# atom501/v-img

Measured on AMD Instinct MI355X. Metric: Mrays/sec (primary+secondary) at 512 spp, higher is better.
Workload: dtype f32; 1 GPU; disney_spheres.json, mis integrator, 512 spp, 1800x800; integrator=mis, spp=512, depth=unbounded, bvh=sweep SAH (host)

## Files before the change

### v-img_amd/csrc/device_scene.h

```cpp
#pragma once
#include <hip/hip_runtime.h>
#include <stdint.h>

#include "../../include/vimg_scene.h"

namespace vimg {

#define VIMG_GLOBAL __attribute__((address_space(1)))
#define VIMG_LDS __attribute__((address_space(3)))
template <typename T>
using gptr = const VIMG_GLOBAL T*;
typedef float v4f __attribute__((ext_vector_type(4)));
typedef uint32_t v2u __attribute__((ext_vector_type(2)));
typedef uint32_t v4u __attribute__((ext_vector_type(4)));

struct __attribute__((aligned(16))) DNode {
  v4f a;
  v4f b;
  v4f c;
  uint32_t left_ref, right_ref, pad0, pad1;
};
static_assert(sizeof(DNode) == 64, "DNode must be one 64-byte line");

struct __attribute__((aligned(16))) DLeafPrim {
  v4f a, b;
  float c0;
  uint32_t prim;
// ... 18 lines not shown

struct DScene {
  float cam_to_world[16];
  float p_size0, p_size1;
  float cone_spread;
  float aperture_radius, focal_dist;
  int32_t res_x, res_y;

  float root_min[3], root_max[3];
  uint32_t num_nodes, max_depth;
  uint32_t root_ref;
  gptr<DNode> nodes;
  gptr<DLeafPrim> leaf_prims;

  gptr<VimgPrim> prims;
  gptr<DTriShade> tri_shade;
  gptr<float> tri_area_pdf;
  gptr<VimgMesh> meshes;
  gptr<float> normals;
  gptr<float> uvs;
  gptr<VimgSphere> spheres;
  gptr<VimgMaterial> materials;
  gptr<uint32_t> material_flags;
  gptr<VimgTexture> textures;
  gptr<float> texels;
  gptr<VimgTextureRG> rg_textures;
  gptr<float> rg_texels;
  gptr<VimgLight> lights;
  gptr<DLight> dlights;
  uint32_t num_lights;
  gptr<float> cdf_pool;
  VimgBackground background;
  uint32_t background_emissive;
};

enum : uint32_t {
  MATF_NEEDS_UV = 1u,
  MATF_NEEDS_FRAME = 2u,
};

struct RenderArgs {
  uint32_t integrator, samples, depth;
  uint32_t tile_rank, tile_world;
  uint32_t tiles_x, tiles_y;
  uint32_t num_local_tiles;
  uint32_t full_stats;
// ... 49 lines not shown
```

### v-img_amd/csrc/hip_internal.h

```cpp
#pragma once
#include <hip/hip_runtime.h>

#include <algorithm>
#include <string>
#include <utility>
#include <vector>

#include "../../include/vimg_hip.h"
#include "device_mem.h"
#include "device_scene.h"
#include "kernel_tus.h"

#pragma GCC visibility push(hidden)
struct VimgDeviceScene {
  vimg::DScene d{};
  vimg::DevBuf nodes, leaf_prims;
  vimg::DevBuf chain_leaf;
  std::vector<vimg::DevBuf> tables;
  size_t total_bytes = 0;
  bool textured = false;
  VimgHipOptions opt{};
  int waves_per_simd = 2;
  bool too_wide = false;
  bool force_general = false;
  uint32_t num_cus = 0;
  uint32_t num_leaf_prims = 0;
  vimg::DevBuf stats;
  vimg::DevBuf counter;
  vimg::DevBuf root_box;
  vimg::DevBuf frame;
  vimg::DevBuf pool_cold;
  vimg::DevBuf stack_ovf;
  vimg::DevBuf pool_state;
  uint32_t pool_epoch = 0;
  uint64_t generation = 0;
  uint32_t num_vertices = 0, num_tris = 0, num_spheres = 0;
  std::vector<std::pair<uint32_t, uint32_t>> normal_rows;
  uint32_t n_internal = 0;
  uint32_t n_chain = 0;
  std::vector<uint32_t> level_begin;
  std::vector<VimgMaterial> materials;
  std::vector<VimgTexture> textures;
  std::vector<VimgLight> lights;
  uint32_t num_rg_textures = 0;
  uint64_t num_texels = 0, num_cdf = 0;
  size_t lights_table = 0, dlights_table = 0;
  int query_launch = -1;
  bool query_ready = false;
  vimg::RenderArgs query_args{};
  uint32_t query_lds = 0;
  uint32_t query_per_cu[3] = {0, 0, 0};
};

struct VimgProgressive {
  VimgDeviceScene* scene = nullptr;
  VimgRenderParams params{};
  uint64_t items = 0;
  vimg::DevBuf rec[2];
  int cur = 0;
  uint32_t samples = 0;
  vimg::DevBuf scratch;
  uint64_t generation = 0;
  bool uniform = true;
  uint64_t valid_items = 0;
  uint64_t launches = 0;
  vimg::DevBuf item_list;
  vimg::DevBuf block_counts;
  vimg::DevBuf ctl;
};
// ... 17 lines not shown
  bool deep;
  int cu_waves;
  bool feature;
  size_t cold_bytes;
  size_t ovf_bytes;
};

struct DeviceTree {
  DevBuf nodes, bb, obj_indices;
  uint32_t num_nodes = 0, max_depth = 0;
  std::vector<uint32_t> level_internal;
};
int build_tree_device(uint32_t builder , uint32_t n, const float* d_bounds6, DeviceTree* out);

int validate_materials(const VimgMaterial* materials, uint32_t num_materials, const VimgTexture* textures, uint32_t num_textures,
                       uint32_t num_rg_textures);
int validate_lights(const VimgLight* lights, uint32_t num_lights, uint32_t num_prims);
bool tables_textured(const VimgMaterial* materials, uint32_t num_materials, const VimgTexture* textures, const VimgBackground& bg);
bool background_is_emissive(const VimgBackground& bg);

struct RelightPlan {
  bool any = false;
  DevBuf new_lights, new_dlights;
  DevBuf sin_elev, lum, row_int, row_tot;
  std::vector<float> sin_table;
};
int check_relight(const VimgDeviceScene* s, const VimgGeometryUpdate* u);
int prepare_relight(const VimgDeviceScene* s, const VimgGeometryUpdate* u, RelightPlan* plan);
int enqueue_relight(VimgDeviceScene* s, const VimgGeometryUpdate* u, RelightPlan* plan, hipStream_t st);
void commit_relight(VimgDeviceScene* s, const VimgGeometryUpdate* u, RelightPlan* plan);

struct EnvCdfScratch {
  float* sin_elev;
  float* lum;
  float* row_int;
  float* row_tot;
};
void enqueue_mip_levels(float* texels, const uint64_t* level_offset, uint32_t levels, uint32_t w, uint32_t h, uint32_t wrap_u,
                        uint32_t wrap_v, hipStream_t st);
std::vector<float> env_sin_table(uint32_t h);
void enqueue_env_cdfs(const float* img, uint32_t w, uint32_t h, const EnvCdfScratch& t, float* row_cdf, float* col_cdfs, hipStream_t st);

struct ProgLaunch {
  uint32_t base;
  const void* in;
  void* out;
  const uint32_t* item_list = nullptr;
  uint32_t item_count = 0;
  bool keep_stats = false;
};
int check_params(const VimgDeviceScene* s, const VimgRenderParams* p);
int check_render(const VimgDeviceScene* s, const VimgRenderParams* p, const void* d_out);
struct RenderLaunch {
// ... 25 lines not shown
```

### v-img_amd/csrc/render_kernels.h

```cpp
#pragma once
#include "device_math.h"
#include "device_scene.h"

namespace vimg {


struct Rng {
  uint64_t s;
};
VD uint32_t pcg_next(Rng& r) {
  uint64_t old = r.s;
  r.s = old * 6364136223846793005ULL + 1ULL;
  uint32_t xorshifted = static_cast<uint32_t>(((old >> 18u) ^ old) >> 27u);
  uint32_t rot = static_cast<uint32_t>(old >> 59u);
  return (xorshifted >> rot) | (xorshifted << ((0u - rot) & 31u));
}
VD void pcg_seed(Rng& r, uint64_t initstate) {
  r.s = 0;
  pcg_next(r);
  r.s += initstate;
  pcg_next(r);
}
constexpr uint64_t kPcgA = 6364136223846793005ULL;
constexpr uint64_t pcg_a_pow(int n) { uint64_t r = 1; for (int i = 0; i < n; ++i) r *= kPcgA; return r; }
constexpr uint64_t pcg_c_sum(int n) { uint64_t r = 0; for (int i = 0; i < n; ++i) r += pcg_a_pow(i); return r; }
// ... 736 lines not shown
}

enum : uint32_t {
  LOBE_NONE = 0,
  LOBE_COSINE = 1,
  LOBE_CLEARCOAT = 2,
  LOBE_METAL = 3,
  LOBE_GLASS = 4,
  LOBE_DIELECTRIC = 5
};

VD float fresnel_dielectric(float n_dot_i, float eta) {
  float n_dot_t_sq = 1.f - (1.f - n_dot_i * n_dot_i) / (eta * eta);
  if (n_dot_t_sq < 0) return 1;
  float n_dot_t = sqrt_f(n_dot_t_sq);
  n_dot_i = absf(n_dot_i);
  float rs = (n_dot_i - eta * n_dot_t) / (n_dot_i + eta * n_dot_t);
  float rp = (eta * n_dot_i - n_dot_t) / (eta * n_dot_i + n_dot_t);
  return (rs * rs + rp * rp) / 2;
}
VD float fd_term(f3 n, f3 w, float fd90) {
  return 1.f + (fd90 - 1.f) * pow5(1.f - sel_max(dot(n, w), 0.f));
}
VD void regularize_alpha(float& ax, float& ay) {
  ax = ax < 0.1f ? clampf(2.f * ax, 0.03f, 0.1f) : ax;
  ay = ay < 0.1f ? clampf(2.f * ay, 0.03f, 0.1f) : ay;
}

struct PrincipledCommon {
  f3 dir_in;
  Onb frame;
  float metallic, roughness;
};
template <bool TEX>
VD PrincipledCommon principled_prologue(const DScene& g, gptr<VimgMaterial> m, f3 wi, const Hit& hit) {
  PrincipledCommon p;
  p.dir_in = -wi;
  p.frame = Onb{hit.tu, hit.tv, hit.ns};
  if ((dot(hit.ns, p.dir_in) * dot(hit.ng, p.dir_in)) < 0) {
    p.frame.u = -p.frame.u;
    p.frame.v = -p.frame.v;
    p.frame.w = -p.frame.w;
  }
  f2 m_r{1.f, 1.f};
  if constexpr (TEX) {
    if (m->mr_tex >= 0) m_r = rg_get_at_uv(g, m->mr_tex, hit.mr_uv);
  }
  m_r = m_r * f2{m->metallic_factor, m->roughness_factor};
  p.metallic = m_r.x;
  p.roughness = m_r.y;
  return p;
}

template <bool TEX>
VD void principled_eval_pdf(const DScene& g, gptr<VimgMaterial> m, f3 wi,
                                                 f3 wo, const Hit& hit, RayCone cone,
                                                 bool regularize, f3& f_out, float& pdf_out) {
  const PrincipledCommon pc = principled_prologue<TEX>(g, m, wi, hit);
  const f3 dir_in = pc.dir_in;
  const Onb& frame = pc.frame;
  const float metallic = pc.metallic, roughness = pc.roughness;
  const f3 base_color = col_at_ray_hit<TEX>(g, m->tex, wi, cone, hit);
  const f3 half_vector = normalize(dir_in + wo);
  constexpr float alpha_min = 0.0001;
  const float aspect = sqrt_f(1.f - 0.9f * m->anisotropic);
  const float roughness_clamp = clampf(roughness, 0.01f, 1.f);
  const float roughness_square = roughness_clamp * roughness_clamp;
  float alphax = sel_max(alpha_min, roughness_square / aspect);
  float alphay = sel_max(alpha_min, roughness_square * aspect);
  if (regularize) regularize_alpha(alphax, alphay);
  const float g_in = g_w(dir_in, alphax, alphay, frame);
  const float G = g_in * g_w(wo, alphax, alphay, frame);
  const float ng_in = dot(hit.ng, dir_in);
  const float ng_out = dot(hit.ng, wo);

  f3 eval_glass;
  float pdf_glass;
  {
    const float mat_eta = m->eta;
    float in_geo_dot = dot(dir_in, hit.ng);
    bool reflect = (in_geo_dot * dot(hit.ng, wo)) >= 0;
    float eta = in_geo_dot >= 0 ? mat_eta : 1.f / mat_eta;
    f3 hv = half_vector;
    if (!reflect) hv = normalize(dir_in + wo * eta);
    float h_dot_in = dot(hv, dir_in);
    float F = fresnel_dielectric(h_dot_in, eta);
    const f3 lh = project_onto_onb(frame, hv);
    float had = (lh.x * lh.x) / (alphax * alphax) + (lh.y * lh.y) / (alphay * alphay)
                + (lh.z * lh.z);
    float D = 1. / (kPi * alphax * alphay * (had * had));
    float normal_in_dot = dot(frame.w, dir_in);
    if (reflect) {
      eval_glass = base_color * (F * D * G) / (4.f * absf(normal_in_dot));
      pdf_glass = (F * D * g_in) / (4.f * absf(normal_in_dot));
    } else {
      float eta_factor = 1.f / (eta * eta);
      float h_dot_out = dot(hv, wo);
      float sqrt_denom = h_dot_in + eta * h_dot_out;
      eval_glass = f3{sqrt_f(base_color.x), sqrt_f(base_color.y), sqrt_f(base_color.z)}
                   * (eta_factor * (1 - F) * D * G * eta * eta * absf(h_dot_out * h_dot_in))
                   / (absf(normal_in_dot) * sqrt_denom * sqrt_denom);
      float dh_dout = eta * eta * h_dot_out / (sqrt_denom * sqrt_denom);
      pdf_glass = (1.f - F) * D * g_in * absf(dh_dout * h_dot_in / normal_in_dot);
    }
  }
  const float st = m->specular_transmission;
  if (ng_in < 0) {
    f_out = (1.f - metallic) * st * eval_glass;
    pdf_out = pdf_glass;
    return;
  }
  const bool below = (ng_in < 0 || ng_out < 0);

  f3 eval_sheen{0.f, 0.f, 0.f};
  f3 eval_diff{0.f, 0.f, 0.f};
  float pdf_diff = 0.f;
  f3 eval_clearcoat{0.f, 0.f, 0.f};
  float pdf_clearcoat = 0.f;
  f3 eval_metal{0.f, 0.f, 0.f};
  float pdf_metal = 0.f;

  float alpha_g = (1.f - m->clearcoat_gloss) * 0.1f + m->clearcoat_gloss * 0.001f;
  alpha_g = regularize && (alpha_g < 0.1f) ? clampf(2.f * alpha_g, 0.03f, 0.1f) : alpha_g;

  if (!below) {
    const float base_lum = luminance(base_color);
    const f3 c_tint = base_lum > 0 ? base_color / base_lum : splat3(1.f);
    {
      const float sheen_tint = m->sheen_tint;
      f3 c_sheen = (splat3(1.f) - splat3(sheen_tint)) + sheen_tint * c_tint;
      eval_sheen = c_sheen * pow5(1.f - sel_max(dot(half_vector, wo), 0.f))
                   * sel_max(dot(frame.w, wo), 0.f);
    }
    {
      const float subsurface = m->subsurface;
      float normal_dirout_dot = dot(frame.w, wo);
      const float cos_theta_out = sel_max(normal_dirout_dot, 0.f);
      const float cos_theta_in = sel_max(dot(frame.w, dir_in), 0.f);
      const float dot_h_out = sel_max(dot(half_vector, wo), 0.f);
      const float fd90 = 0.5 + 2.0 * roughness * dot_h_out * dot_h_out;
      const f3 base_diffuse = base_color * kInvPiF * fd_term(frame.w, dir_in, fd90)
                              * fd_term(frame.w, wo, fd90) * cos_theta_out;
      const float fss90 = roughness * dot_h_out * dot_h_out;
      f3 ss_diffuse = base_color * 1.25f * kInvPiF
                      * (fd_term(frame.w, dir_in, fss90) * fd_term(frame.w, wo, fss90)
                             * ((1.f / (cos_theta_out + cos_theta_in)) - 0.5f)
                         + 0.5f)
                      * cos_theta_out;
      eval_diff = (1.f - subsurface) * base_diffuse + subsurface * ss_diffuse;
      pdf_diff = sel_max(normal_dirout_dot, 0.f) * kInvPiF;
    }
    {
      constexpr float R0 = ((1.5f - 1.f) * (1.5f - 1.f)) / ((1.5f + 1.f) * (1.5f + 1.f));
      float h_dirout_dot = absf(dot(half_vector, wo));
      float fresnel = R0 + (1. - R0) * pow5(1.f - h_dirout_dot);
      float Gc = g_w(dir_in, 0.25, 0.25, frame) * g_w(wo, 0.25, 0.25, frame);
      const float ag2 = alpha_g * alpha_g;
      const f3 lh = project_onto_onb(frame, half_vector);
      float D = (ag2 - 1.f) / (kPi * F_log(ag2) * (1. + (ag2 - 1.) * lh.z * lh.z));
      float clearcoat_eval = (fresnel * D * Gc) / (4.f * absf(dot(frame.w, dir_in)));
      pdf_clearcoat = (D * absf(dot(frame.w, half_vector))) / (4.f * h_dirout_dot);
      eval_clearcoat = splat3(clearcoat_eval);
    }
    {
      const float spec_tint = m->specular_tint, specular = m->specular, eta = m->eta;
      f3 k_s = (splat3(1.f) - splat3(spec_tint)) + spec_tint * c_tint;
      float R0 = ((eta - 1.f) * (eta - 1.f)) / ((eta + 1.f) * (eta + 1.f));
      f3 c_0 = (specular * R0 * (1.f - metallic)) * k_s + metallic * base_color;
      f3 fresnel = c_0 + (splat3(1.f) - c_0) * pow5(1.f - dot(half_vector, wo));
      const f3 lh = project_onto_onb(frame, half_vector);
      float had = (lh.x * lh.x) / (alphax * alphax) + (lh.y * lh.y) / (alphay * alphay)
                  + (lh.z * lh.z);
      float D = 1. / (kPi * alphax * alphay * (had * had));
      float d_mul_denominator = D / (4.f * absf(dot(frame.w, dir_in)));
      eval_metal = fresnel * G * d_mul_denominator;
      pdf_metal = g_in * d_mul_denominator;
    }
  }
  const float clearcoat = m->clearcoat, sheen = m->sheen;
  f3 eval_principled = ((1.f - st) * (1.f - metallic) * eval_diff)
                       + ((1.f - metallic) * sheen * eval_sheen)
                       + (0.25f * clearcoat * eval_clearcoat)
                       + ((1.f - st * (1.f - metallic)) * eval_metal)
                       + ((1.f - metallic) * st * eval_glass);
  float diffuse_weight = (1.f - metallic) * (1.f - st);
  float clearcoat_weight = 0.25f * clearcoat;
  float metal_weight = (1.f - st * (1.f - metallic));
  float glass_weight = (1.f - metallic) * st;
  float total_w = diffuse_weight + clearcoat_weight + metal_weight + glass_weight;
  float choose_diff = diffuse_weight / total_w;
  float choose_clearcoat = clearcoat_weight / total_w;
  float choose_metal = metal_weight / total_w;
  float choose_glass = glass_weight / total_w;
  pdf_out = choose_diff * pdf_diff + choose_clearcoat * pdf_clearcoat + choose_metal * pdf_metal
            + choose_glass * pdf_glass;
  f_out = eval_principled;
}

template <bool TEX, int MT = -1>
VD Scatter sample_mat(const DScene& g, const Hit& hit, f3 wi, Rng& rng, bool regularize) {
  gptr<VimgMaterial> m = g.materials + hit.mat;
  const uint32_t type = MT >= 0 ? uint32_t(MT) : m->type;
  const f3 dir_in = -wi;
  uint32_t lobe = LOBE_NONE;
  Onb frame{f3{1.f, 0.f, 0.f}, f3{0.f, 1.f, 0.f}, f3{0.f, 0.f, 1.f}};
  float alphax = 0.f, alphay = 0.f, eta = 0.f, alpha_g = 0.f;
  bool lambert_front = true;

  if (type == VIMG_MAT_LAMBERTIAN) {
    lobe = LOBE_COSINE;
    lambert_front = dot(wi, hit.ns) < 0;
    frame = init_onb(lambert_front ? hit.ns : -hit.ns);
  } else if (type == VIMG_MAT_DIELECTRIC) {
    lobe = LOBE_DIELECTRIC;
  } else if (type == VIMG_MAT_PRINCIPLED) {
    const PrincipledCommon pc = principled_prologue<TEX>(g, m, wi, hit);
    frame = pc.frame;
    const float metallic = pc.metallic;
    float roughness = pc.roughness;
    const float ng_in = dot(hit.ng, dir_in);
    if (ng_in < 0) {
      lobe = LOBE_GLASS;
    } else {
      const float st = m->specular_transmission;
      float diffuse_weight = (1.f - metallic) * (1.f - st);
      float clearcoat_weight = 0.25f * m->clearcoat;
      float metal_weight = (1.f - st * (1.f - metallic));
      float glass_weight = (1.f - metallic) * st;
      float total_w = diffuse_weight + clearcoat_weight + metal_weight + glass_weight;
      float choose_diff = diffuse_weight / total_w;
      float choose_clearcoat = clearcoat_weight / total_w;
      float choose_metal = metal_weight / total_w;
      float choose_glass = glass_weight / total_w;
      float rnd = rand_float(rng);
      if (rnd <= choose_diff) {
        lobe = LOBE_COSINE;
      } else if (rnd > choose_diff && rnd <= (choose_diff + choose_clearcoat)) {
        lobe = LOBE_CLEARCOAT;
      } else if (rnd > (choose_diff + choose_clearcoat)
                 && rnd <= (choose_diff + choose_clearcoat + choose_metal)) {
        lobe = LOBE_METAL;
      } else if (rnd > (choose_diff + choose_clearcoat + choose_metal)
                 && rnd <= (choose_diff + choose_clearcoat + choose_metal + choose_glass)) {
        lobe = LOBE_GLASS;
      }
    }
    if (lobe == LOBE_CLEARCOAT) {
      const float gloss = m->clearcoat_gloss;
      alpha_g = (1.f - gloss) * 0.1f + gloss * 0.001f;
      if (regularize && alpha_g < 0.1f) alpha_g = clampf(2.f * alpha_g, 0.03f, 0.1f);
    } else if (lobe == LOBE_METAL || lobe == LOBE_GLASS) {
      constexpr float alpha_min = 0.0001;
      float aspect = sqrt_f(1.f - 0.9f * m->anisotropic);
      if (lobe == LOBE_GLASS) roughness = clampf(roughness, 0.01f, 1.f);
      float roughness_square = roughness * roughness;
      alphax = sel_max(alpha_min, roughness_square / aspect);
      alphay = sel_max(alpha_min, roughness_square * aspect);
      if (regularize) regularize_alpha(alphax, alphay);
      const float mat_eta = m->eta;
      eta = ng_in >= 0 ? mat_eta : 1.f / mat_eta;
    }
  }
  if (lobe == LOBE_DIELECTRIC) return dielectric_sample(m, hit, wi, rng);
  if (lobe == LOBE_NONE) return no_scatter();

  const float ra = rand_float(rng);
  const float rb = rand_float(rng);
  const float phi = 2 * kPi * ((lobe == LOBE_CLEARCOAT) ? rb : ra);
  double sin_phi, cos_phi;
  sincos_azimuth(phi, sin_phi, cos_phi);

  if (lobe == LOBE_COSINE) {
    float cos_theta = sqrt_f(rb);
    float sin_theta = sqrt_f(1 - cos_theta * cos_theta);
    f3 local{static_cast<float>(cos_phi) * sin_theta, static_cast<float>(sin_phi) * sin_theta,
             cos_theta};
    f3 dir = xform_with_onb(frame, local);
    if (type == VIMG_MAT_LAMBERTIAN) {
      if (lambert_front) return Scatter{dir, 0.f, false, true};
      return no_scatter();
    }
    if (dot(hit.ng, dir) <= 0) return no_scatter();
    return Scatter{dir, 0.f, false, true};
// ... 45 lines not shown
  if (rnd <= F) {
    f3 reflected = normalize(-dir_in + 2 * dot(dir_in, half_vec) * half_vec);
    if (dot(reflected, hit.ng) * dot(dir_in, hit.ng) <= 0) return no_scatter();
    return Scatter{reflected, 0.f, true, true};
  }
  float h_dot_out_sq = 1 - (1 - h_dot_in * h_dot_in) / (eta * eta);
  if (h_dot_out_sq <= 0) return no_scatter();
  if (h_dot_in < 0) half_vec = -half_vec;
  float h_dot_out = static_cast<float>(__builtin_sqrt(static_cast<double>(h_dot_out_sq)));
  f3 refracted = -dir_in / eta + (absf(h_dot_in) / eta - h_dot_out) * half_vec;
  if (dot(refracted, hit.ng) * dot(dir_in, hit.ng) >= 0) return no_scatter();
  f3 generalized_h = normalize(dir_in + refracted * eta);
  float g_h_dot_in = dot(generalized_h, dir_in);
  if ((1 - (1 - g_h_dot_in * g_h_dot_in) / (eta * eta)) <= 0) return no_scatter();
  return Scatter{refracted, eta, true, true};
}
template <bool TEX, int MT = -1>
VD void eval_pdf_pair(const DScene& g, const Hit& hit, f3 wi, f3 wo, RayCone cone, bool regularize,
                      f3& f, float& pdf) {
  gptr<VimgMaterial> m = g.materials + hit.mat;
  const uint32_t type = MT >= 0 ? uint32_t(MT) : m->type;
  if (type == VIMG_MAT_LAMBERTIAN) {
    float dot_product = static_cast<float>(sel_max(0.0f, dot(wo, hit.ns)) / kPi);
    f = col_at_ray_hit<TEX>(g, m->tex, wi, cone, hit) * dot_product;
    pdf = dot_product;
  } else if (type == VIMG_MAT_PRINCIPLED) {
    principled_eval_pdf<TEX>(g, m, wi, wo, hit, cone, regularize, f, pdf);
  } else {
    f = f3{0.f, 0.f, 0.f};
    pdf = 1.0f;
  }
}

VD void tri_light_sample_with(f3 p0, f3 p1, f3 p2, f3 n0, f3 n1, f3 n2, float pdf, f3 look_from, Rng& rng, f3& hit_n,
                              EmitterInfo& info) {
  float rand1 = rand_float(rng);
  float rand2 = rand_float(rng);
  float u, v;
  if (rand1 < rand2) {
    u = rand1 / 2.f;
    v = rand2 - u;
  } else {
    v = rand2 / 2.f;
    u = rand1 - v;
  }
  float w = 1.f - u - v;
  const f3 hit_p = p0 * u + p1 * v + p2 * w;
// ... 630 lines not shown
```

### v-img_amd/csrc/scene_relight.hip

```cpp
#include <hip/hip_runtime.h>

#include <cstring>

#include "device_math.h"
#include "hip_internal.h"
#include "scene_bake.h"

namespace vimg {

namespace {

constexpr uint32_t kBlock = 256;

template <typename T>
VD T* flat(gptr<T> p) {
  return (T*)p;
}

dim3 blocks_for(uint32_t n) { return dim3((n + kBlock - 1) / kBlock); }

}

__global__ void __launch_bounds__(kBlock) scene_relight_flags(const DScene d, uint32_t num_materials) {
  const uint32_t i = blockIdx.x * blockDim.x + threadIdx.x;
  if (i >= num_materials) return;
  flat(d.material_flags)[i] = bake_material_flags(flat(d.materials)[i], flat(d.textures));
}

__global__ void __launch_bounds__(kBlock) scene_relight_cls(const DScene d, uint32_t num_slots) {
  const uint32_t j = blockIdx.x * blockDim.x + threadIdx.x;
  if (j >= num_slots) return;
  DLeafPrim* lp = flat(d.leaf_prims) + j;
  const VimgPrim p = flat(d.prims)[lp->prim];
  lp->cls = bake_material_class(flat(d.materials)[bake_prim_material(p, flat(d.tri_shade), flat(d.meshes), flat(d.spheres))].type);
}

__global__ void __launch_bounds__(kBlock)
scene_relight_lights(const DScene d, const VimgLight* __restrict__ lights, uint32_t num_lights, DLight* __restrict__ out) {
  const uint32_t i = blockIdx.x * blockDim.x + threadIdx.x;
  if (i >= num_lights) return;
  out[i] = bake_light(lights[i], flat(d.prims), flat(d.tri_shade), flat(d.tri_area_pdf), flat(d.meshes), flat(d.spheres), flat(d.materials));
}

namespace {

bool is_env_image(const VimgBackground& bg, uint32_t texture) {
  return bg.type == VIMG_BG_ENVMAP && bg.env_tex >= 0 && static_cast<uint32_t>(bg.env_tex) == texture;
}

bool levels_disjoint(const VimgTexture& t) {
  for (uint32_t a = 0; a < t.num_levels; ++a)
    for (uint32_t b = a + 1; b < t.num_levels; ++b) {
      const uint64_t na = uint64_t(std::max(t.width >> a, 1u)) * std::max(t.height >> a, 1u);
      const uint64_t nb = uint64_t(std::max(t.width >> b, 1u)) * std::max(t.height >> b, 1u);
      if (t.level_offset[a] < t.level_offset[b] + nb && t.level_offset[b] < t.level_offset[a] + na) return false;
    }
  return true;
}

}

int check_relight(const VimgDeviceScene* s, const VimgGeometryUpdate* u) {
  const uint32_t num_textures = static_cast<uint32_t>(s->textures.size());
  if (u->textures)
// ... 22 lines not shown
    if (backgrounds > 1) return fail(VIMG_E_INVALID, "update: more than one background entry in lights");
  }
  if (u->num_images && !u->images) return fail(VIMG_E_INVALID, "update: num_images without images");
  for (uint32_t k = 0; k < u->num_images; ++k) {
    const VimgTextureImage& im = u->images[k];
    if (im.texture >= num_textures || s->textures[im.texture].type != VIMG_TEX_IMAGE)
      return fail(VIMG_E_INVALID, "update: images: texture is not a resident image texture");
    if (!im.level0 || (reinterpret_cast<uintptr_t>(im.level0) & 3u))
      return fail(VIMG_E_INVALID, "update: images: level0 is null or not 4-byte aligned");
    if (!levels_disjoint(s->textures[im.texture]))
      return fail(VIMG_E_UNSUPPORTED, "update: images: the texture's mip levels overlap in the texel pool");
  }
  return VIMG_OK;
}

int prepare_relight(const VimgDeviceScene* s, const VimgGeometryUpdate* u, RelightPlan* plan) {
  plan->any = u->materials || u->textures || u->set_lights || u->background || u->num_images;
  if (!plan->any) return VIMG_OK;
  if (g_device < 0) return fail(VIMG_E_DEVICE, "update: no device");
  if (u->set_lights) {
    if (int rc = plan->new_lights.alloc(std::max<size_t>(u->num_lights, 1) * sizeof(VimgLight))) return rc;
    if (int rc = plan->new_dlights.alloc(std::max<size_t>(u->num_lights, 1) * sizeof(DLight))) return rc;
  }
  for (uint32_t k = 0; k < u->num_images; ++k)
    if (is_env_image(s->d.background, u->images[k].texture) && !plan->lum.p) {
      const VimgTexture& t = s->textures[u->images[k].texture];
      plan->sin_table = env_sin_table(t.height);
      if (int rc = plan->sin_elev.alloc(size_t(t.height) * sizeof(float))) return rc;
      if (int rc = plan->lum.alloc(size_t(t.width) * t.height * sizeof(float))) return rc;
      if (int rc = plan->row_int.alloc(size_t(t.height) * sizeof(float))) return rc;
      if (int rc = plan->row_tot.alloc(sizeof(float))) return rc;
    }
  return VIMG_OK;
}

int enqueue_relight(VimgDeviceScene* s, const VimgGeometryUpdate* u, RelightPlan* plan, hipStream_t st) {
  const DScene& d = s->d;
  float* texels = (float*)d.texels;
  float* cdf_pool = (float*)d.cdf_pool;
  for (uint32_t k = 0; k < u->num_images; ++k) {
    const VimgTextureImage& im = u->images[k];
    const VimgTexture& t = s->textures[im.texture];
    float* level0 = texels + t.level_offset[0] * 3;
    HIP_TRY(hipMemcpyAsync(level0, im.level0, size_t(t.width) * t.height * 3 * sizeof(float), hipMemcpyDeviceToDevice, st));
    enqueue_mip_levels(texels, t.level_offset, t.num_levels, t.width, t.height, t.wrap_u, t.wrap_v, st);
    if (is_env_image(d.background, im.texture)) {
      HIP_TRY(hipMemcpyAsync(plan->sin_elev.p, plan->sin_table.data(), plan->sin_table.size() * sizeof(float), hipMemcpyHostToDevice, st));
      enqueue_env_cdfs(level0, t.width, t.height,
                       EnvCdfScratch{plan->sin_elev.as<float>(), plan->lum.as<float>(), plan->row_int.as<float>(), plan->row_tot.as<float>()},
                       cdf_pool + d.background.row_cdf_offset, cdf_pool + d.background.col_cdf_offset, st);
    }
  }
  if (u->textures && !s->textures.empty())
    HIP_TRY(hipMemcpyAsync((void*)d.textures, u->textures, s->textures.size() * sizeof(VimgTexture), hipMemcpyHostToDevice, st));
  if (u->materials && !s->materials.empty()) {
    const uint32_t n = static_cast<uint32_t>(s->materials.size());
    HIP_TRY(hipMemcpyAsync((void*)d.materials, u->materials, size_t(n) * sizeof(VimgMaterial), hipMemcpyHostToDevice, st));
    hipLaunchKernelGGL(scene_relight_flags, blocks_for(n), dim3(kBlock), 0, st, d, n);
    hipLaunchKernelGGL(scene_relight_cls, blocks_for(s->num_leaf_prims), dim3(kBlock), 0, st, d, s->num_leaf_prims);
  }
  if (u->set_lights) {
    if (u->num_lights) {
      HIP_TRY(hipMemcpyAsync(plan->new_lights.p, u->lights, size_t(u->num_lights) * sizeof(VimgLight), hipMemcpyHostToDevice, st));
      hipLaunchKernelGGL(scene_relight_lights, blocks_for(u->num_lights), dim3(kBlock), 0, st, d, plan->new_lights.as<const VimgLight>(),
                         u->num_lights, plan->new_dlights.as<DLight>());
    }
  } else if (u->materials && d.num_lights) {
    hipLaunchKernelGGL(scene_relight_lights, blocks_for(d.num_lights), dim3(kBlock), 0, st, d, (const VimgLight*)d.lights, d.num_lights,
                       (DLight*)d.dlights);
  }
  HIP_TRY(hipGetLastError());
  return VIMG_OK;
}

void commit_relight(VimgDeviceScene* s, const VimgGeometryUpdate* u, RelightPlan* plan) {
  DScene& d = s->d;
  if (u->textures) s->textures.assign(u->textures, u->textures + s->textures.size());
  if (u->materials) s->materials.assign(u->materials, u->materials + s->materials.size());
  if (u->background) {
    d.background = *u->background;
    d.background_emissive = background_is_emissive(d.background);
  }
  s->textured = tables_textured(s->materials.data(), static_cast<uint32_t>(s->materials.size()), s->textures.data(), d.background);
  if (u->set_lights) {
    DevBuf& lights = s->tables[s->lights_table];
    DevBuf& dlights = s->tables[s->dlights_table];
    s->total_bytes = s->total_bytes - lights.bytes - dlights.bytes + plan->new_lights.bytes + plan->new_dlights.bytes;
    lights = std::move(plan->new_lights);
    dlights = std::move(plan->new_dlights);
    d.lights = (decltype(d.lights))lights.p;
    d.dlights = (decltype(d.dlights))dlights.p;
    d.num_lights = u->num_lights;
    s->lights.assign(u->lights, u->lights + u->num_lights);
    s->waves_per_simd = (s->total_bytes > (32u << 20)) ? 3 : 2;
  }
}

}
```

### v-img_amd/csrc/scene_upload.hip

```cpp
#include <cmath>
#include <cstdlib>
#include <cstring>
#include <memory>
#include <numbers>

#include "hip_internal.h"
#include "scene_bake.h"
#include "scene_update.h"

using namespace vimg;

namespace {

template <typename T>
int upload(VimgDeviceScene* s, DevBuf& b, const T* host, size_t count) {
  if (int rc = b.alloc(std::max<size_t>(count, 1) * sizeof(T))) return rc;
  s->total_bytes += b.bytes;
  if (count) HIP_TRY(hipMemcpy(b.p, host, count * sizeof(T), hipMemcpyHostToDevice));
  return VIMG_OK;
}

}

int vimg::validate_materials(const VimgMaterial* materials, uint32_t num_materials, const VimgTexture* textures, uint32_t num_textures,
// ... 333 lines not shown
  UP_TO(s->nodes, nodes, t.nodes.data(), t.nodes.size());
  UP_TO(s->leaf_prims, leaf_prims, leaf.data(), leaf.size());
  s->num_leaf_prims = static_cast<uint32_t>(leaf.size());
  UP(prims, sc->prims, sc->num_prims);
  UP(tri_shade, shade.data(), shade.size());
  UP(tri_area_pdf, area_pdf.data(), area_pdf.size());
  UP(meshes, sc->meshes, sc->num_meshes);
  UP(normals, sc->normals, size_t(sc->num_vertices) * 3);
  UP(uvs, sc->uvs, sc->num_uvs * 2);
  UP(spheres, sc->spheres, sc->num_spheres);
  UP(materials, sc->materials, sc->num_materials);
  UP(material_flags, mflags.data(), mflags.size());
  UP(textures, sc->textures, sc->num_textures);
  UP(texels, sc->texels, sc->num_texels * 3);
  UP(rg_textures, sc->rg_textures, sc->num_rg_textures);
  UP(rg_texels, sc->rg_texels, sc->num_rg_texels * 2);
  UP(lights, sc->lights, sc->num_lights);
  s->lights_table = s->tables.size() - 1;
  UP(dlights, dlights.data(), dlights.size());
  s->dlights_table = s->tables.size() - 1;
  UP(cdf_pool, sc->cdf_pool, sc->num_cdf);
#undef UP
#undef UP_TO
  if (!t.chain_leaf.empty()) {
    if (int rc = s->chain_leaf.alloc(t.chain_leaf.size() * sizeof(uint32_t))) return rc;
    HIP_TRY(hipMemcpy(s->chain_leaf.p, t.chain_leaf.data(), s->chain_leaf.bytes, hipMemcpyHostToDevice));
  }
  return VIMG_OK;
}

void record_for_updates(VimgDeviceScene* s, const VimgScene* sc) {
  s->materials.assign(sc->materials, sc->materials + sc->num_materials);
  s->textures.assign(sc->textures, sc->textures + sc->num_textures);
  s->lights.assign(sc->lights, sc->lights + sc->num_lights);
  s->num_rg_textures = sc->num_rg_textures;
  s->num_texels = sc->num_texels;
  s->num_cdf = sc->num_cdf;
  s->num_vertices = sc->num_vertices;
  s->num_tris = sc->num_tris;
  s->num_spheres = sc->num_spheres;
  for (uint32_t i = 0; i < sc->num_meshes; ++i) {
    const VimgMesh& m = sc->meshes[i];
    if (!m.has_normals || m.num_vertices == 0) continue;
    auto& r = s->normal_rows;
    if (!r.empty() && r.back().first + r.back().second == m.first_vertex)
      r.back().second += m.num_vertices;
// ... 150 lines not shown
```

Baseline: 14750 Mrays/s.

## Precompute per-material BSDF constants into a baked device material table

Adds a DMaterial record holding per-material derived terms (alphas, coat terms, lobe weights, eta terms, constant-colour tints). A bake kernel fills it at upload and on relight. The principled eval and sample paths read these precomputed values instead of recomputing them from raw material parameters and texture lookups on every bounce. This trades ALU work and texture fetches for extra global loads from a 304-byte record per hit. It also adds register and code pressure in the shading path.

```diff
diff --git a/v-img_amd/csrc/device_scene.h b/v-img_amd/csrc/device_scene.h
--- a/v-img_amd/csrc/device_scene.h
+++ b/v-img_amd/csrc/device_scene.h
@@ -3,6 +3,7 @@
 #include <stdint.h>
 
 #include "../../include/vimg_scene.h"
+#include "material_record.h"
 
 namespace vimg {
 
@@ -67,6 +68,7 @@
   gptr<VimgSphere> spheres;
   gptr<VimgMaterial> materials;
   gptr<uint32_t> material_flags;
+  gptr<DMaterial> dmaterials;
   gptr<VimgTexture> textures;
   gptr<float> texels;
   gptr<VimgTextureRG> rg_textures;
diff --git a/v-img_amd/csrc/hip_internal.h b/v-img_amd/csrc/hip_internal.h
--- a/v-img_amd/csrc/hip_internal.h
+++ b/v-img_amd/csrc/hip_internal.h
@@ -44,7 +44,7 @@
   std::vector<VimgLight> lights;
   uint32_t num_rg_textures = 0;
   uint64_t num_texels = 0, num_cdf = 0;
-  size_t lights_table = 0, dlights_table = 0;
+  size_t lights_table = 0, dlights_table = 0, dmaterials_table = 0;
   int query_launch = -1;
   bool query_ready = false;
   vimg::RenderArgs query_args{};
@@ -108,6 +108,7 @@
 struct RelightPlan {
   bool any = false;
   DevBuf new_lights, new_dlights;
+  DevBuf new_dmaterials;
   DevBuf sin_elev, lum, row_int, row_tot;
   std::vector<float> sin_table;
 };
@@ -115,6 +116,7 @@
 int prepare_relight(const VimgDeviceScene* s, const VimgGeometryUpdate* u, RelightPlan* plan);
 int enqueue_relight(VimgDeviceScene* s, const VimgGeometryUpdate* u, RelightPlan* plan, hipStream_t st);
 void commit_relight(VimgDeviceScene* s, const VimgGeometryUpdate* u, RelightPlan* plan);
+int enqueue_material_bake(const DScene& d, uint32_t num_materials, DMaterial* out, hipStream_t st);
 
 struct EnvCdfScratch {
   float* sin_elev;
diff --git a/v-img_amd/csrc/material_record.h b/v-img_amd/csrc/material_record.h
--- /dev/null
+++ b/v-img_amd/csrc/material_record.h
@@ -0,0 +1,69 @@
+#pragma once
+#include <stdint.h>
+
+#include "../../include/vimg_scene.h"
+
+#if defined(__HIP__) || defined(__CUDACC__)
+#define VIMG_HD __host__ __device__ inline
+#else
+#define VIMG_HD inline
+#endif
+
+namespace vimg {
+
+struct DMatAlpha {
+  float ax, ay;
+  float ax2, ay2;
+  double pi_axay;
+};
+struct DMatCoat {
+  float alpha_g, ag2;
+  float ag2m1;
+  float pad;
+  double ag2m1_d;
+  double pi_log;
+};
+struct DMatEta {
+  float eta, eta2, inv_eta2;
+  float pad;
+};
+struct DMatWeights {
+  float choose_diff, choose_clearcoat, choose_metal, choose_glass;
+  float sum2, sum3, sum4;
+  float mix_diff, mix_sheen, mix_coat, mix_metal, mix_glass;
+};
+
+enum : uint32_t {
+  DMAT_SCALARS = 1u,
+  DMAT_COLOUR = 2u,
+};
+
+struct __attribute__((aligned(16))) DMaterial {
+  uint32_t bits;
+  float r0;
+  float spec_r0;
+  float pad0;
+  DMatWeights w;
+  DMatAlpha alpha[2];
+  float salpha[2][2];
+  DMatCoat coat[2];
+  DMatEta eta[2];
+  float base[3];
+  float c_sheen[3], k_s[3];
+  float c_0[3], one_minus_c_0[3];
+  float sqrt_base[3];
+  float pad1[2];
+};
+static_assert(sizeof(DMatAlpha) == 24 && sizeof(DMatCoat) == 32 && sizeof(DMatEta) == 16 && sizeof(DMatWeights) == 48,
+              "DMaterial's groups have fixed sizes");
+static_assert(sizeof(DMaterial) == 304 && alignof(DMaterial) == 16, "DMaterial must be 304 bytes, 16-byte aligned");
+
+VIMG_HD uint32_t dmaterial_bits(const VimgMaterial& m, const VimgTexture* textures) {
+  uint32_t b = 0;
+  if (m.type == VIMG_MAT_PRINCIPLED && m.mr_tex < 0) b |= DMAT_SCALARS;
+  if ((m.type == VIMG_MAT_PRINCIPLED || m.type == VIMG_MAT_LAMBERTIAN) && m.tex >= 0 && textures[m.tex].type == VIMG_TEX_CONST)
+    b |= DMAT_COLOUR;
+  return b;
+}
+
+}
diff --git a/v-img_amd/csrc/material_terms.h b/v-img_amd/csrc/material_terms.h
--- /dev/null
+++ b/v-img_amd/csrc/material_terms.h
@@ -0,0 +1,123 @@
+#pragma once
+#include "device_math.h"
+#include "material_record.h"
+
+namespace vimg {
+
+VD void regularize_alpha(float& ax, float& ay) {
+  ax = ax < 0.1f ? clampf(2.f * ax, 0.03f, 0.1f) : ax;
+  ay = ay < 0.1f ? clampf(2.f * ay, 0.03f, 0.1f) : ay;
+}
+
+VD void mat_alphas(float roughness, float anisotropic, bool regularize, float& alphax, float& alphay) {
+  constexpr float alpha_min = 0.0001;
+  const float aspect = sqrt_f(1.f - 0.9f * anisotropic);
+  const float roughness_square = roughness * roughness;
+  alphax = sel_max(alpha_min, roughness_square / aspect);
+  alphay = sel_max(alpha_min, roughness_square * aspect);
+  if (regularize) regularize_alpha(alphax, alphay);
+}
+VD DMatAlpha mat_alpha_terms(float roughness, float anisotropic, bool regularize) {
+  DMatAlpha a;
+  mat_alphas(roughness, anisotropic, regularize, a.ax, a.ay);
+  a.ax2 = a.ax * a.ax;
+  a.ay2 = a.ay * a.ay;
+  a.pi_axay = kPi * a.ax * a.ay;
+  return a;
+}
+
+VD float mat_alpha_g(float gloss, bool regularize) {
+  float alpha_g = (1.f - gloss) * 0.1f + gloss * 0.001f;
+  alpha_g = regularize && (alpha_g < 0.1f) ? clampf(2.f * alpha_g, 0.03f, 0.1f) : alpha_g;
+  return alpha_g;
+}
+VD DMatCoat mat_coat_terms(float gloss, bool regularize) {
+  DMatCoat c;
+  c.alpha_g = mat_alpha_g(gloss, regularize);
+  const float ag2 = c.alpha_g * c.alpha_g;
+  c.ag2 = ag2;
+  c.ag2m1 = (ag2 - 1.f);
+  c.pad = 0.f;
+  c.ag2m1_d = (ag2 - 1.);
+  c.pi_log = kPi * F_log(ag2);
+  return c;
+}
+
+VD DMatEta mat_eta_terms(float mat_eta, bool entering) {
+  DMatEta e;
+  e.eta = entering ? mat_eta : 1.f / mat_eta;
+  e.eta2 = e.eta * e.eta;
+  e.inv_eta2 = 1.f / (e.eta * e.eta);
+  e.pad = 0.f;
+  return e;
+}
+
+VD float mat_r0(float eta) { return ((eta - 1.f) * (eta - 1.f)) / ((eta + 1.f) * (eta + 1.f)); }
+VD float mat_spec_r0(float specular, float R0, float metallic) { return (specular * R0 * (1.f - metallic)); }
+
+VD DMatWeights mat_weight_terms(float metallic, float st, float clearcoat, float sheen) {
+  DMatWeights w;
+  w.mix_diff = (1.f - st) * (1.f - metallic);
+  w.mix_sheen = (1.f - metallic) * sheen;
+  w.mix_coat = 0.25f * clearcoat;
+  w.mix_metal = (1.f - st * (1.f - metallic));
+  w.mix_glass = (1.f - metallic) * st;
+  float diffuse_weight = (1.f - metallic) * (1.f - st);
+  float clearcoat_weight = 0.25f * clearcoat;
+  float metal_weight = (1.f - st * (1.f - metallic));
+  float glass_weight = (1.f - metallic) * st;
+  float total_w = diffuse_weight + clearcoat_weight + metal_weight + glass_weight;
+  w.choose_diff = diffuse_weight / total_w;
+  w.choose_clearcoat = clearcoat_weight / total_w;
+  w.choose_metal = metal_weight / total_w;
+  w.choose_glass = glass_weight / total_w;
+  w.sum2 = (w.choose_diff + w.choose_clearcoat);
+  w.sum3 = (w.choose_diff + w.choose_clearcoat + w.choose_metal);
+  w.sum4 = (w.choose_diff + w.choose_clearcoat + w.choose_metal + w.choose_glass);
+  return w;
+}
+
+VD f3 mat_c_tint(f3 base_color) {
+  const float base_lum = dot(base_color, f3{0.212671f, 0.715160f, 0.072169f});
+  return base_lum > 0 ? base_color / base_lum : splat3(1.f);
+}
+VD f3 mat_c_sheen(f3 c_tint, float sheen_tint) { return (splat3(1.f) - splat3(sheen_tint)) + sheen_tint * c_tint; }
+VD f3 mat_k_s(f3 c_tint, float spec_tint) { return (splat3(1.f) - splat3(spec_tint)) + spec_tint * c_tint; }
+VD f3 mat_c_0(float spec_r0, f3 k_s, float metallic, f3 base_color) { return spec_r0 * k_s + metallic * base_color; }
+VD f3 mat_one_minus(f3 c_0) { return (splat3(1.f) - c_0); }
+VD f3 mat_sqrt3(f3 base_color) { return f3{sqrt_f(base_color.x), sqrt_f(base_color.y), sqrt_f(base_color.z)}; }
+
+VD DMaterial bake_dmaterial(const VimgMaterial& m, uint32_t bits, f3 base_color) {
+  DMaterial r{};
+  r.bits = bits;
+  if (m.type == VIMG_MAT_PRINCIPLED) {
+    const float metallic = 1.f * m.metallic_factor, roughness = 1.f * m.roughness_factor;
+    r.r0 = mat_r0(m.eta);
+    r.spec_r0 = mat_spec_r0(m.specular, r.r0, metallic);
+    r.w = mat_weight_terms(metallic, m.specular_transmission, m.clearcoat, m.sheen);
+    for (int reg = 0; reg < 2; ++reg) {
+      r.alpha[reg] = mat_alpha_terms(clampf(roughness, 0.01f, 1.f), m.anisotropic, reg != 0);
+      mat_alphas(roughness, m.anisotropic, reg != 0, r.salpha[reg][0], r.salpha[reg][1]);
+      r.coat[reg] = mat_coat_terms(m.clearcoat_gloss, reg != 0);
+    }
+    r.eta[0] = mat_eta_terms(m.eta, true);
+    r.eta[1] = mat_eta_terms(m.eta, false);
+  }
+  if (bits & DMAT_COLOUR) {
+    auto put = [](float* dst, f3 v) { dst[0] = v.x, dst[1] = v.y, dst[2] = v.z; };
+    put(r.base, base_color);
+    if (m.type == VIMG_MAT_PRINCIPLED) {
+      const f3 c_tint = mat_c_tint(base_color);
+      const f3 k_s = mat_k_s(c_tint, m.specular_tint);
+      const f3 c_0 = mat_c_0(r.spec_r0, k_s, 1.f * m.metallic_factor, base_color);
+      put(r.c_sheen, mat_c_sheen(c_tint, m.sheen_tint));
+      put(r.k_s, k_s);
+      put(r.c_0, c_0);
+      put(r.one_minus_c_0, mat_one_minus(c_0));
+      put(r.sqrt_base, mat_sqrt3(base_color));
+    }
+  }
+  return r;
+}
+
+}
diff --git a/v-img_amd/csrc/render_kernels.h b/v-img_amd/csrc/render_kernels.h
--- a/v-img_amd/csrc/render_kernels.h
+++ b/v-img_amd/csrc/render_kernels.h
@@ -1,6 +1,7 @@
 #pragma once
 #include "device_math.h"
 #include "device_scene.h"
+#include "material_terms.h"
 
 namespace vimg {
 
@@ -783,9 +784,27 @@
 VD float fd_term(f3 n, f3 w, float fd90) {
   return 1.f + (fd90 - 1.f) * pow5(1.f - sel_max(dot(n, w), 0.f));
 }
-VD void regularize_alpha(float& ax, float& ay) {
-  ax = ax < 0.1f ? clampf(2.f * ax, 0.03f, 0.1f) : ax;
-  ay = ay < 0.1f ? clampf(2.f * ay, 0.03f, 0.1f) : ay;
+
+VD DMatCoat load_coat(gptr<DMatCoat> p) {
+  DMatCoat c;
+  c.alpha_g = p->alpha_g, c.ag2 = p->ag2, c.ag2m1 = p->ag2m1, c.pad = 0.f, c.ag2m1_d = p->ag2m1_d, c.pi_log = p->pi_log;
+  return c;
+}
+VD DMatWeights load_weights(gptr<DMatWeights> p) {
+  DMatWeights w;
+  w.choose_diff = p->choose_diff, w.choose_clearcoat = p->choose_clearcoat, w.choose_metal = p->choose_metal;
+  w.choose_glass = p->choose_glass, w.sum2 = p->sum2, w.sum3 = p->sum3, w.sum4 = p->sum4;
+  w.mix_diff = p->mix_diff, w.mix_sheen = p->mix_sheen, w.mix_coat = p->mix_coat, w.mix_metal = p->mix_metal;
+  w.mix_glass = p->mix_glass;
+  return w;
+}
+VD gptr<DMaterial> dmat_at(const DScene& g, uint32_t mat) {
+  asm volatile("" : "+v"(mat));
+  return g.dmaterials + mat;
+}
+template <bool TEX>
+VD bool dmat_scalars(uint32_t bits) {
+  return !TEX || (bits & DMAT_SCALARS) != 0;
 }
 
 struct PrincipledCommon {
@@ -821,15 +840,31 @@
   const f3 dir_in = pc.dir_in;
   const Onb& frame = pc.frame;
   const float metallic = pc.metallic, roughness = pc.roughness;
-  const f3 base_color = col_at_ray_hit<TEX>(g, m->tex, wi, cone, hit);
+  const uint32_t mat = hit.mat;
+  const int reg = regularize ? 1 : 0;
+  float alphax, alphay;
+  f3 base_color;
+  bool scalars, colour;
+  {
+    gptr<DMaterial> dm = dmat_at(g, mat);
+    const uint32_t bits = dm->bits;
+    scalars = dmat_scalars<TEX>(bits), colour = (bits & DMAT_COLOUR) != 0;
+    base_color = colour ? load3(dm->base) : col_at_ray_hit<TEX>(g, m->tex, wi, cone, hit);
+    if (scalars) {
+      alphax = dm->alpha[reg].ax, alphay = dm->alpha[reg].ay;
+    } else {
+      mat_alphas(clampf(roughness, 0.01f, 1.f), m->anisotropic, regularize, alphax, alphay);
+    }
+  }
+  auto alpha_products = [&](float& ax2, float& ay2, double& pi_axay) {
+    if (scalars) {
+      gptr<DMatAlpha> a = dmat_at(g, mat)->alpha + reg;
+      ax2 = a->ax2, ay2 = a->ay2, pi_axay = a->pi_axay;
+    } else {
+      ax2 = alphax * alphax, ay2 = alphay * alphay, pi_axay = kPi * alphax * alphay;
+    }
+  };
   const f3 half_vector = normalize(dir_in + wo);
-  constexpr float alpha_min = 0.0001;
-  const float aspect = sqrt_f(1.f - 0.9f * m->anisotropic);
-  const float roughness_clamp = clampf(roughness, 0.01f, 1.f);
-  const float roughness_square = roughness_clamp * roughness_clamp;
-  float alphax = sel_max(alpha_min, roughness_square / aspect);
-  float alphay = sel_max(alpha_min, roughness_square * aspect);
-  if (regularize) regularize_alpha(alphax, alphay);
   const float g_in = g_w(dir_in, alphax, alphay, frame);
   const float G = g_in * g_w(wo, alphax, alphay, frame);
   const float ng_in = dot(hit.ng, dir_in);
@@ -838,36 +873,38 @@
   f3 eval_glass;
   float pdf_glass;
   {
-    const float mat_eta = m->eta;
     float in_geo_dot = dot(dir_in, hit.ng);
     bool reflect = (in_geo_dot * dot(hit.ng, wo)) >= 0;
-    float eta = in_geo_dot >= 0 ? mat_eta : 1.f / mat_eta;
+    const DMatEta et = mat_eta_terms(m->eta, in_geo_dot >= 0);
+    float ax2, ay2;
+    double pi_axay;
+    alpha_products(ax2, ay2, pi_axay);
+    const float eta = et.eta;
     f3 hv = half_vector;
     if (!reflect) hv = normalize(dir_in + wo * eta);
     float h_dot_in = dot(hv, dir_in);
     float F = fresnel_dielectric(h_dot_in, eta);
     const f3 lh = project_onto_onb(frame, hv);
-    float had = (lh.x * lh.x) / (alphax * alphax) + (lh.y * lh.y) / (alphay * alphay)
-                + (lh.z * lh.z);
-    float D = 1. / (kPi * alphax * alphay * (had * had));
+    float had = (lh.x * lh.x) / ax2 + (lh.y * lh.y) / ay2 + (lh.z * lh.z);
+    float D = 1. / (pi_axay * (had * had));
     float normal_in_dot = dot(frame.w, dir_in);
     if (reflect) {
       eval_glass = base_color * (F * D * G) / (4.f * absf(normal_in_dot));
       pdf_glass = (F * D * g_in) / (4.f * absf(normal_in_dot));
     } else {
-      float eta_factor = 1.f / (eta * eta);
+      float eta_factor = et.inv_eta2;
       float h_dot_out = dot(hv, wo);
       float sqrt_denom = h_dot_in + eta * h_dot_out;
-      eval_glass = f3{sqrt_f(base_color.x), sqrt_f(base_color.y), sqrt_f(base_color.z)}
+      eval_glass = (colour ? load3(dmat_at(g, mat)->sqrt_base) : mat_sqrt3(base_color))
                    * (eta_factor * (1 - F) * D * G * eta * eta * absf(h_dot_out * h_dot_in))
                    / (absf(normal_in_dot) * sqrt_denom * sqrt_denom);
-      float dh_dout = eta * eta * h_dot_out / (sqrt_denom * sqrt_denom);
+      float dh_dout = et.eta2 * h_dot_out / (sqrt_denom * sqrt_denom);
       pdf_glass = (1.f - F) * D * g_in * absf(dh_dout * h_dot_in / normal_in_dot);
     }
   }
-  const float st = m->specular_transmission;
   if (ng_in < 0) {
-    f_out = (1.f - metallic) * st * eval_glass;
+    const float mix_glass = mat_weight_terms(metallic, m->specular_transmission, m->clearcoat, m->sheen).mix_glass;
+    f_out = mix_glass * eval_glass;
     pdf_out = pdf_glass;
     return;
   }
@@ -881,15 +918,11 @@
   f3 eval_metal{0.f, 0.f, 0.f};
   float pdf_metal = 0.f;
 
-  float alpha_g = (1.f - m->clearcoat_gloss) * 0.1f + m->clearcoat_gloss * 0.001f;
-  alpha_g = regularize && (alpha_g < 0.1f) ? clampf(2.f * alpha_g, 0.03f, 0.1f) : alpha_g;
-
   if (!below) {
-    const float base_lum = luminance(base_color);
-    const f3 c_tint = base_lum > 0 ? base_color / base_lum : splat3(1.f);
+    f3 c_tint{0.f, 0.f, 0.f};
+    if (!colour) c_tint = mat_c_tint(base_color);
     {
-      const float sheen_tint = m->sheen_tint;
-      f3 c_sheen = (splat3(1.f) - splat3(sheen_tint)) + sheen_tint * c_tint;
+      const f3 c_sheen = colour ? load3(dmat_at(g, mat)->c_sheen) : mat_c_sheen(c_tint, m->sheen_tint);
       eval_sheen = c_sheen * pow5(1.f - sel_max(dot(half_vector, wo), 0.f))
                    * sel_max(dot(frame.w, wo), 0.f);
     }
@@ -916,45 +949,37 @@
       float h_dirout_dot = absf(dot(half_vector, wo));
       float fresnel = R0 + (1. - R0) * pow5(1.f - h_dirout_dot);
       float Gc = g_w(dir_in, 0.25, 0.25, frame) * g_w(wo, 0.25, 0.25, frame);
-      const float ag2 = alpha_g * alpha_g;
+      const DMatCoat cc = scalars ? load_coat(dmat_at(g, mat)->coat + reg) : mat_coat_terms(m->clearcoat_gloss, regularize);
       const f3 lh = project_onto_onb(frame, half_vector);
-      float D = (ag2 - 1.f) / (kPi * F_log(ag2) * (1. + (ag2 - 1.) * lh.z * lh.z));
+      float D = cc.ag2m1 / (cc.pi_log * (1. + cc.ag2m1_d * lh.z * lh.z));
       float clearcoat_eval = (fresnel * D * Gc) / (4.f * absf(dot(frame.w, dir_in)));
       pdf_clearcoat = (D * absf(dot(frame.w, half_vector))) / (4.f * h_dirout_dot);
       eval_clearcoat = splat3(clearcoat_eval);
     }
     {
-      const float spec_tint = m->specular_tint, specular = m->specular, eta = m->eta;
-      f3 k_s = (splat3(1.f) - splat3(spec_tint)) + spec_tint * c_tint;
-      float R0 = ((eta - 1.f) * (eta - 1.f)) / ((eta + 1.f) * (eta + 1.f));
-      f3 c_0 = (specular * R0 * (1.f - metallic)) * k_s + metallic * base_color;
-      f3 fresnel = c_0 + (splat3(1.f) - c_0) * pow5(1.f - dot(half_vector, wo));
+      const f3 k_s = colour ? load3(dmat_at(g, mat)->k_s) : mat_k_s(c_tint, m->specular_tint);
+      const f3 c_0 = mat_c_0(mat_spec_r0(m->specular, mat_r0(m->eta), metallic), k_s, metallic, base_color);
+      const f3 one_minus_c_0 = mat_one_minus(c_0);
+      f3 fresnel = c_0 + one_minus_c_0 * pow5(1.f - dot(half_vector, wo));
       const f3 lh = project_onto_onb(frame, half_vector);
-      float had = (lh.x * lh.x) / (alphax * alphax) + (lh.y * lh.y) / (alphay * alphay)
-                  + (lh.z * lh.z);
-      float D = 1. / (kPi * alphax * alphay * (had * had));
+      float ax2, ay2;
+      double pi_axay;
+      alpha_products(ax2, ay2, pi_axay);
+      float had = (lh.x * lh.x) / ax2 + (lh.y * lh.y) / ay2 + (lh.z * lh.z);
+      float D = 1. / (pi_axay * (had * had));
       float d_mul_denominator = D / (4.f * absf(dot(frame.w, dir_in)));
       eval_metal = fresnel * G * d_mul_denominator;
       pdf_metal = g_in * d_mul_denominator;
     }
   }
-  const float clearcoat = m->clearcoat, sheen = m->sheen;
-  f3 eval_principled = ((1.f - st) * (1.f - metallic) * eval_diff)
-                       + ((1.f - metallic) * sheen * eval_sheen)
-                       + (0.25f * clearcoat * eval_clearcoat)
-                       + ((1.f - st * (1.f - metallic)) * eval_metal)
-                       + ((1.f - metallic) * st * eval_glass);
-  float diffuse_weight = (1.f - metallic) * (1.f - st);
-  float clearcoat_weight = 0.25f * clearcoat;
-  float metal_weight = (1.f - st * (1.f - metallic));
-  float glass_weight = (1.f - metallic) * st;
-  float total_w = diffuse_weight + clearcoat_weight + metal_weight + glass_weight;
-  float choose_diff = diffuse_weight / total_w;
-  float choose_clearcoat = clearcoat_weight / total_w;
-  float choose_metal = metal_weight / total_w;
-  float choose_glass = glass_weight / total_w;
-  pdf_out = choose_diff * pdf_diff + choose_clearcoat * pdf_clearcoat + choose_metal * pdf_metal
-            + choose_glass * pdf_glass;
+  const DMatWeights w = mat_weight_terms(metallic, m->specular_transmission, m->clearcoat, m->sheen);
+  f3 eval_principled = (w.mix_diff * eval_diff)
+                       + (w.mix_sheen * eval_sheen)
+                       + (w.mix_coat * eval_clearcoat)
+                       + (w.mix_metal * eval_metal)
+                       + (w.mix_glass * eval_glass);
+  pdf_out = w.choose_diff * pdf_diff + w.choose_clearcoat * pdf_clearcoat + w.choose_metal * pdf_metal
+            + w.choose_glass * pdf_glass;
   f_out = eval_principled;
 }
 
@@ -980,46 +1005,36 @@
     const float metallic = pc.metallic;
     float roughness = pc.roughness;
     const float ng_in = dot(hit.ng, dir_in);
+    gptr<DMaterial> dm = g.dmaterials + hit.mat;
+    const bool scalars = dmat_scalars<TEX>(dm->bits);
+    const int reg = regularize ? 1 : 0;
     if (ng_in < 0) {
       lobe = LOBE_GLASS;
     } else {
-      const float st = m->specular_transmission;
-      float diffuse_weight = (1.f - metallic) * (1.f - st);
-      float clearcoat_weight = 0.25f * m->clearcoat;
-      float metal_weight = (1.f - st * (1.f - metallic));
-      float glass_weight = (1.f - metallic) * st;
-      float total_w = diffuse_weight + clearcoat_weight + metal_weight + glass_weight;
-      float choose_diff = diffuse_weight / total_w;
-      float choose_clearcoat = clearcoat_weight / total_w;
-      float choose_metal = metal_weight / total_w;
-      float choose_glass = glass_weight / total_w;
+      const DMatWeights w = scalars ? load_weights(&dm->w) : mat_weight_terms(metallic, m->specular_transmission, m->clearcoat, m->sheen);
       float rnd = rand_float(rng);
-      if (rnd <= choose_diff) {
+      if (rnd <= w.choose_diff) {
         lobe = LOBE_COSINE;
-      } else if (rnd > choose_diff && rnd <= (choose_diff + choose_clearcoat)) {
+      } else if (rnd > w.choose_diff && rnd <= w.sum2) {
         lobe = LOBE_CLEARCOAT;
-      } else if (rnd > (choose_diff + choose_clearcoat)
-                 && rnd <= (choose_diff + choose_clearcoat + choose_metal)) {
+      } else if (rnd > w.sum2 && rnd <= w.sum3) {
         lobe = LOBE_METAL;
-      } else if (rnd > (choose_diff + choose_clearcoat + choose_metal)
-                 && rnd <= (choose_diff + choose_clearcoat + choose_metal + choose_glass)) {
+      } else if (rnd > w.sum3 && rnd <= w.sum4) {
         lobe = LOBE_GLASS;
       }
     }
     if (lobe == LOBE_CLEARCOAT) {
-      const float gloss = m->clearcoat_gloss;
-      alpha_g = (1.f - gloss) * 0.1f + gloss * 0.001f;
-      if (regularize && alpha_g < 0.1f) alpha_g = clampf(2.f * alpha_g, 0.03f, 0.1f);
+      alpha_g = scalars ? dm->coat[reg].alpha_g : mat_alpha_g(m->clearcoat_gloss, regularize);
     } else if (lobe == LOBE_METAL || lobe == LOBE_GLASS) {
-      constexpr float alpha_min = 0.0001;
-      float aspect = sqrt_f(1.f - 0.9f * m->anisotropic);
-      if (lobe == LOBE_GLASS) roughness = clampf(roughness, 0.01f, 1.f);
-      float roughness_square = roughness * roughness;
-      alphax = sel_max(alpha_min, roughness_square / aspect);
-      alphay = sel_max(alpha_min, roughness_square * aspect);
-      if (regularize) regularize_alpha(alphax, alphay);
-      const float mat_eta = m->eta;
-      eta = ng_in >= 0 ? mat_eta : 1.f / mat_eta;
+      if (scalars) {
+        alphax = lobe == LOBE_GLASS ? dm->alpha[reg].ax : dm->salpha[reg][0];
+        alphay = lobe == LOBE_GLASS ? dm->alpha[reg].ay : dm->salpha[reg][1];
+        eta = dm->eta[ng_in >= 0 ? 0 : 1].eta;
+      } else {
+        if (lobe == LOBE_GLASS) roughness = clampf(roughness, 0.01f, 1.f);
+        mat_alphas(roughness, m->anisotropic, regularize, alphax, alphay);
+        eta = mat_eta_terms(m->eta, ng_in >= 0).eta;
+      }
     }
   }
   if (lobe == LOBE_DIELECTRIC) return dielectric_sample(m, hit, wi, rng);
@@ -1111,7 +1126,9 @@
   const uint32_t type = MT >= 0 ? uint32_t(MT) : m->type;
   if (type == VIMG_MAT_LAMBERTIAN) {
     float dot_product = static_cast<float>(sel_max(0.0f, dot(wo, hit.ns)) / kPi);
-    f = col_at_ray_hit<TEX>(g, m->tex, wi, cone, hit) * dot_product;
+    gptr<DMaterial> dm = g.dmaterials + hit.mat;
+    const f3 col = (dm->bits & DMAT_COLOUR) ? load3(dm->base) : col_at_ray_hit<TEX>(g, m->tex, wi, cone, hit);
+    f = col * dot_product;
     pdf = dot_product;
   } else if (type == VIMG_MAT_PRINCIPLED) {
     principled_eval_pdf<TEX>(g, m, wi, wo, hit, cone, regularize, f, pdf);
diff --git a/v-img_amd/csrc/scene_relight.hip b/v-img_amd/csrc/scene_relight.hip
--- a/v-img_amd/csrc/scene_relight.hip
+++ b/v-img_amd/csrc/scene_relight.hip
@@ -4,6 +4,7 @@
 
 #include "device_math.h"
 #include "hip_internal.h"
+#include "material_terms.h"
 #include "scene_bake.h"
 
 namespace vimg {
@@ -40,6 +41,26 @@
   const uint32_t i = blockIdx.x * blockDim.x + threadIdx.x;
   if (i >= num_lights) return;
   out[i] = bake_light(lights[i], flat(d.prims), flat(d.tri_shade), flat(d.tri_area_pdf), flat(d.meshes), flat(d.spheres), flat(d.materials));
+}
+
+__global__ void __launch_bounds__(kBlock) scene_bake_materials(const DScene d, uint32_t num_materials, DMaterial* __restrict__ out) {
+  const uint32_t i = blockIdx.x * blockDim.x + threadIdx.x;
+  if (i >= num_materials) return;
+  const VimgMaterial m = flat(d.materials)[i];
+  const uint32_t bits = dmaterial_bits(m, flat(d.textures));
+  f3 base{0.f, 0.f, 0.f};
+  if (bits & DMAT_COLOUR) {
+    const VimgTexture* t = flat(d.textures) + m.tex;
+    base = f3{t->col_a[0], t->col_a[1], t->col_a[2]};
+  }
+  out[i] = bake_dmaterial(m, bits, base);
+}
+
+int enqueue_material_bake(const DScene& d, uint32_t num_materials, DMaterial* out, hipStream_t st) {
+  if (!num_materials) return VIMG_OK;
+  hipLaunchKernelGGL(scene_bake_materials, blocks_for(num_materials), dim3(kBlock), 0, st, d, num_materials, out);
+  HIP_TRY(hipGetLastError());
+  return VIMG_OK;
 }
 
 namespace {
@@ -108,6 +129,8 @@
     if (int rc = plan->new_lights.alloc(std::max<size_t>(u->num_lights, 1) * sizeof(VimgLight))) return rc;
     if (int rc = plan->new_dlights.alloc(std::max<size_t>(u->num_lights, 1) * sizeof(DLight))) return rc;
   }
+  if ((u->materials || u->textures) && !s->materials.empty())
+    if (int rc = plan->new_dmaterials.alloc(s->materials.size() * sizeof(DMaterial))) return rc;
   for (uint32_t k = 0; k < u->num_images; ++k)
     if (is_env_image(s->d.background, u->images[k].texture) && !plan->lum.p) {
       const VimgTexture& t = s->textures[u->images[k].texture];
@@ -145,6 +168,8 @@
     hipLaunchKernelGGL(scene_relight_flags, blocks_for(n), dim3(kBlock), 0, st, d, n);
     hipLaunchKernelGGL(scene_relight_cls, blocks_for(s->num_leaf_prims), dim3(kBlock), 0, st, d, s->num_leaf_prims);
   }
+  if (plan->new_dmaterials.p)
+    if (int rc = enqueue_material_bake(d, static_cast<uint32_t>(s->materials.size()), plan->new_dmaterials.as<DMaterial>(), st)) return rc;
   if (u->set_lights) {
     if (u->num_lights) {
       HIP_TRY(hipMemcpyAsync(plan->new_lights.p, u->lights, size_t(u->num_lights) * sizeof(VimgLight), hipMemcpyHostToDevice, st));
@@ -166,6 +191,11 @@
   if (u->background) {
     d.background = *u->background;
     d.background_emissive = background_is_emissive(d.background);
+  }
+  if (plan->new_dmaterials.p) {
+    DevBuf& dmaterials = s->tables[s->dmaterials_table];
+    dmaterials = std::move(plan->new_dmaterials);
+    d.dmaterials = (decltype(d.dmaterials))dmaterials.p;
   }
   s->textured = tables_textured(s->materials.data(), static_cast<uint32_t>(s->materials.size()), s->textures.data(), d.background);
   if (u->set_lights) {
diff --git a/v-img_amd/csrc/scene_upload.hip b/v-img_amd/csrc/scene_upload.hip
--- a/v-img_amd/csrc/scene_upload.hip
+++ b/v-img_amd/csrc/scene_upload.hip
@@ -379,6 +379,15 @@
   UP(cdf_pool, sc->cdf_pool, sc->num_cdf);
 #undef UP
 #undef UP_TO
+  {
+    DevBuf& b = s->tables.emplace_back();
+    if (int rc = b.alloc(std::max<size_t>(sc->num_materials, 1) * sizeof(DMaterial))) return rc;
+    s->total_bytes += b.bytes;
+    s->dmaterials_table = s->tables.size() - 1;
+    d.dmaterials = (decltype(d.dmaterials))b.p;
+    if (int rc = enqueue_material_bake(d, sc->num_materials, b.as<DMaterial>(), nullptr)) return rc;
+    HIP_TRY(hipStreamSynchronize(nullptr));
+  }
   if (!t.chain_leaf.empty()) {
     if (int rc = s->chain_leaf.alloc(t.chain_leaf.size() * sizeof(uint32_t))) return rc;
     HIP_TRY(hipMemcpy(s->chain_leaf.p, t.chain_leaf.data(), s->chain_leaf.bytes, hipMemcpyHostToDevice));
```

After: 15150 Mrays/s (median of 6 runs). 1.03x the previous value.
